# Terence-23/RayTracing-in-a-weekend

Measured on AMD Instinct MI355X. Metric: Msamples/s (rays x bounces) at 1920x1080x500spp, higher is better.
Workload: dtype f32

## Files before the change

bindings/rust/src/lib.rs:

```rust
use std::os::raw::c_void;

#[repr(C)] #[derive(Clone, Copy, Default)]
pub struct RtwCamera { pub origin: [f32; 3], pub u: [f32; 3], pub v: [f32; 3], pub pixel00: [f32; 3],
    pub delta_u: [f32; 3], pub delta_v: [f32; 3], pub lens_radius: f32, pub time0: f32, pub shutter: f32 }

#[repr(C)] #[derive(Clone, Copy, Default)]
pub struct RtwSphere { pub center: [f32; 3], pub radius: f32, pub velocity: [f32; 3], pub col_mod: [f32; 3],
    pub tex_color: [f32; 3], pub metallicness: f32, pub opacity: f32, pub ir: f32, pub emitted: [f32; 3], pub tex: i32 }

#[repr(C)] #[derive(Clone, Copy, Default)]
pub struct RtwTexture { pub row: u32, pub col: u32, pub texel_offset: u32, pub emit_tex: u32 }

#[repr(C)] #[derive(Clone, Copy, Default)]
pub struct RtwQuad { pub origin: [f32; 3], pub u: [f32; 3], pub v: [f32; 3], pub velocity: [f32; 3], pub tex_color: [f32; 3],
    pub metallicness: f32, pub opacity: f32, pub ir: f32, pub emitted: [f32; 3], pub tex: i32 }

#[repr(C)] #[derive(Clone, Copy, Default)]
pub struct RtwTriangle { pub origin: [f32; 3], pub u: [f32; 3], pub v: [f32; 3], pub normal: [f32; 3], pub d: f32, pub w: [f32; 3],
    pub tex_color: [f32; 3], pub metallicness: f32, pub opacity: f32, pub ir: f32, pub emitted: [f32; 3], pub tex: i32 }

#[repr(C)] #[derive(Clone, Copy, Default)]
pub struct RtwMeshInstance { pub position: [f32; 3], pub quat: [f32; 4] }
pub const RTW_MAX_MESH_INSTANCES: u32 = 65536;
pub type MeshHits = (Vec<f32>, Vec<i32>, Vec<i32>, Vec<[f32; 3]>);
// ... 31 lines not shown
    pub total_ms: f32, pub taps: u64 }
#[repr(C)] #[derive(Clone, Copy, Default)]
pub struct RtwGuidedFilter { pub base: RtwBilateral, pub sigma_depth: f32, pub sigma_normal: f32, pub same_object: u32 }
#[repr(u32)] #[derive(Clone, Copy)]
pub enum ProximityKind { Square = 0, Edges = 1 }
#[derive(Clone, Copy)]
pub struct Proximity { pub size: u32, pub kind: ProximityKind }
impl Proximity { pub fn new(size: u32, kind: ProximityKind) -> Self { Self { size, kind } } }

#[repr(C)] pub struct RtwCtx { _private: [u8; 0] }
#[repr(C)] pub struct RtwMgpu { _private: [u8; 0] }

#[repr(u32)] #[derive(Clone, Copy)]
pub enum Integrator { Gradient = 0, BgColor = 1, Normal = 2, Flag = 3, Rust2 = 4, LightCast = 5, LightBiased = 6 }
#[repr(C)] #[derive(Clone, Copy)]
pub struct RtwLight { pub kind: u32, pub index: u32 }
pub const RTW_MAX_LIGHTS: usize = 16;
pub const RTW_FLAG_MIXED_MATERIAL: u32 = 32;
#[repr(u32)] #[derive(Clone, Copy)]
pub enum Sampler { Row = 0, Stratified = 1, Centres = 2, NoRand = 3 }

pub const RTW_OPT_MESH_LIST_MAX: u32 = 12;
pub const RTW_OPT_MESH_CLIMB: u32 = 13;
#[repr(C)]
#[derive(Clone, Copy, Debug, Default)]
pub struct RtwTriNode { pub lo: [f32; 3], pub skip: u32, pub hi: [f32; 3], pub leaf: u32 }

#[repr(C)]
#[derive(Clone, Copy, Debug, Default)]
pub struct RtwSweepRecord { pub a: u32, pub b: u32, pub got: u32, pub reserved: u32 }
#[repr(C)]
#[derive(Clone, Copy, Debug, Default)]
pub struct RtwSweepResult {
    pub tested: u64, pub wrong: u64, pub n_records: u32, pub reserved: u32, pub records: [RtwSweepRecord; 16], pub kernel_ms: f32, pub reserved2: u32,
}
pub const RTW_MATH_SQRT_PLAIN: (u32, u32, u32) = (0, 1, 1);
pub const RTW_MATH_SQRT_IEEE: (u32, u32, u32) = (1, 1, 1);
pub const RTW_MATH_DIV: (u32, u32, u32) = (2, 2, 1);
pub const RTW_MATH_UNIT: (u32, u32, u32) = (3, 3, 3);
pub const RTW_MATH_UNIT_BALL: (u32, u32, u32) = (4, 4, 3);
pub const RTW_MATH_SPHERE_ROOT: (u32, u32, u32) = (5, 4, 1);
pub const RTW_MATH_ATAN2: (u32, u32, u32) = (6, 2, 1);
pub const RTW_MATH_ACOS: (u32, u32, u32) = (7, 1, 1);
pub const RTW_MATH_SPHERE_UV: (u32, u32, u32) = (8, 3, 2);
pub const RTW_MATH_LN: (u32, u32, u32) = (9, 1, 1);
pub const RTW_MATH_POW: (u32, u32, u32) = (10, 2, 1);
// ... 392 lines not shown
```

include/rtw.h:

```cpp
#ifndef RTW_H
#define RTW_H

#include <stdint.h>
#include <stddef.h>

#ifdef __cplusplus
extern "C" {
#endif

#define RTW_ABI_VERSION 4

#define RTW_OK              0
#define RTW_E_INVALID      -1
#define RTW_E_NO_DEVICE    -2
#define RTW_E_HIP          -3
#define RTW_E_NOMEM        -4
#define RTW_E_UNSUPPORTED  -5
#define RTW_E_NO_SCENE     -6
#define RTW_E_INTERNAL     -7
#define RTW_E_RUNTIME_CONFLICT -8

enum {
    RTW_INTEGRATOR_GRADIENT = 0,
    RTW_INTEGRATOR_BG_COLOR = 1,
// ... 147 lines not shown
int  rtw_ctx_set_stream(rtw_ctx *ctx, void *hip_stream);
int  rtw_ctx_set_scene(rtw_ctx *ctx, const RtwScene *scene, float t_begin, float t_end);
int  rtw_ctx_render(rtw_ctx *ctx, const RtwCamera *cam, const RtwParams *params,
                    float *out_rgb, RtwStats *stats);
int  rtw_ctx_render_multi(rtw_ctx *ctx, const RtwCamera *cam, const RtwParams *params, float fps,
                          uint32_t start_frame, uint32_t n_frames, float *out_rgb, RtwStats *stats);
int  rtw_render(const RtwCamera *cam, const RtwScene *scene, const RtwParams *params,
                float *out_rgb, RtwStats *stats);

enum {
    RTW_OPT_CHUNK_LEN        = 1,
    RTW_OPT_SAMPLE_BANK_GB   = 2,
    RTW_OPT_LDS_GEOM         = 3,
    RTW_OPT_BLOCKS_PER_CU    = 4,
    RTW_OPT_LIST_WALK_MAX    = 5,
    RTW_OPT_TILE_ORDER       = 6,
    RTW_OPT_GRAB_BLOCKS      = 7,
    RTW_OPT_TAIL_UNITS       = 9,
    RTW_OPT_SUB_QUEUES       = 8,
    RTW_OPT_GUIDED_LAYOUT    = 10,
    RTW_OPT_NODE_FORMAT      = 11,
    RTW_OPT_MESH_LIST_MAX    = 12,
    RTW_OPT_MESH_CLIMB       = 13,
};
int  rtw_ctx_set_option(rtw_ctx *ctx, uint32_t key, double value);
int  rtw_ctx_last_render_build(rtw_ctx *ctx, char *buf, size_t n);
int  rtw_ctx_last_node_format(rtw_ctx *ctx);
typedef struct RtwRenderFacts {
    uint32_t integrator, sampler, depth, flags, has_textures;
    uint32_t n_quads, n_instances, noise, n_triangles, rotations, placements;
} RtwRenderFacts;
typedef struct RtwTreeFacts { uint32_t n_nodes, depth, n_spheres, has_f16, has_planes; } RtwTreeFacts;
typedef struct RtwRenderChoice {
    char build[32];
    uint32_t node_format, block, lds_stack_off, lds_geom_off, lds_tri_off, lds_bytes;
} RtwRenderChoice;
int  rtw_render_choice(const RtwRenderFacts *request, const RtwTreeFacts *tree, int32_t opt_lds_geom, uint32_t opt_node_format,
                       uint32_t moving, uint32_t accel, RtwRenderChoice *out);

typedef struct rtw_mgpu rtw_mgpu;
int  rtw_mgpu_create(const int *devices, uint32_t n_devices, rtw_mgpu **out);
void rtw_mgpu_destroy(rtw_mgpu *m);
int  rtw_mgpu_set_scene(rtw_mgpu *m, const RtwScene *scene, float t_begin, float t_end);
int  rtw_mgpu_set_option(rtw_mgpu *m, uint32_t key, double value);
int  rtw_mgpu_render(rtw_mgpu *m, const RtwCamera *cam, const RtwParams *params, float *out_rgb,
                     RtwStats *per_device, RtwStats *total);
int  rtw_render_multi_gpu(const int *devices, uint32_t n_devices, const RtwCamera *cam, const RtwScene *scene,
                          const RtwParams *params, float *out_rgb, RtwStats *per_device);

typedef struct RtwPerlin {
    float   ranvec[256][3];
    uint8_t perm_x[256], perm_y[256], perm_z[256];
} RtwPerlin;
typedef struct RtwTextureNoise {
    int32_t perlin;
    float   scale;
} RtwTextureNoise;
int rtw_perlin_new(uint64_t seed, RtwPerlin *out);
int rtw_perlin_eval(const RtwPerlin *t, const float *points, uint32_t n, uint32_t turb_depth, float *out);
int rtw_ctx_perlin_eval(rtw_ctx *ctx, const RtwPerlin *t, const float *points, uint32_t n, uint32_t turb_depth, float *out);
int rtw_ctx_set_texture_noise(rtw_ctx *ctx, const RtwPerlin *tables, uint32_t n_tables,
// ... 231 lines not shown
```

raytracing-in-a-weekend_amd/__init__.py:

```python
from __future__ import annotations

import ctypes as C
import os
from typing import Optional, Sequence

import numpy as np

_HERE = os.path.dirname(os.path.abspath(__file__))
LIB_PATH = os.environ.get("RTW_HIP_LIB", os.path.join(_HERE, "librtw_hip.so"))

RTW_OK = 0
INTEGRATOR_GRADIENT, INTEGRATOR_BG_COLOR, INTEGRATOR_NORMAL, INTEGRATOR_FLAG, INTEGRATOR_RUST2 = 0, 1, 2, 3, 4
INTEGRATOR_LIGHT_CAST, INTEGRATOR_LIGHT_BIASED = 5, 6
LIGHT_SPHERE, LIGHT_QUAD = 0, 1
MAX_LIGHTS = 16
MAX_MESH_INSTANCES = 65536
SAMPLER_ROW, SAMPLER_STRATIFIED, SAMPLER_CENTRES, SAMPLER_NO_RAND = 0, 1, 2, 3
ACCEL_BRUTE, ACCEL_BVH = 0, 1
FLAG_RECURSIVE_ORDER, FLAG_CPP_DIELECTRIC, FLAG_GLOBAL_NODES, FLAG_CPP_DIFFUSE, FLAG_CHUNK_SUMS = 1, 2, 4, 8, 16
FLAG_CPP = FLAG_CPP_DIELECTRIC | FLAG_CPP_DIFFUSE
FLAG_MIXED_MATERIAL = 32
OPT_CHUNK_LEN, OPT_SAMPLE_BANK_GB, OPT_LDS_GEOM, OPT_BLOCKS_PER_CU, OPT_LIST_WALK_MAX, OPT_TILE_ORDER, OPT_GRAB_BLOCKS, OPT_SUB_QUEUES = 1, 2, 3, 4, 5, 6, 7, 8
OPT_TAIL_UNITS = 9
OPT_NODE_FORMAT = 11
NODE_FORMAT_NONE, NODE_FORMAT_F16, NODE_FORMAT_F32 = 0, 1, 2
OPT_MESH_CLIMB = 13
OPT_MESH_LIST_MAX = 12
MESH_LIST_MAX_DEFAULT = 16
OPT_GUIDED_LAYOUT = 10
SCENE_C1, SCENE_C2, SCENE_C4, SCENE_C5, SCENE_METAL_TEST, SCENE_QUAD_TEST, SCENE_PRESENTATION, SCENE_FIRST_FRAME = 1, 2, 4, 5, 6, 7, 8, 9
MEDIUM_SURFACE, MEDIUM_CONST_DENSITY = 0, 1
PROXIMITY_SQUARE, PROXIMITY_EDGES = 0, 1
PIXELS_U8, PIXELS_F32_RUST2 = 0, 1
BILATERAL_MAX_SIZE = 64
STREAM_LEGACY = 1

METALLIC_M = (1.0, 0.0, 1.0)
SCATTER_M = (0.0, 0.0, 1.0)
FUZZY3_M = (0.7, 0.0, 1.0)
GLASS_M = (1.0, 1.0, 1.5)
GLASSR_M = (1.0, 1.0, float(np.float32(1.0) / np.float32(1.5)))
EMPTY_M = SCATTER_M


class RtwError(RuntimeError):
    def __init__(self, status: int, what: str):
        super().__init__(f"{what}: status {status} ({_strerror(status)})")
        self.status = status


class RtwCamera(C.Structure):
# ... 81 lines not shown
class RtwGuidedFilter(C.Structure):
    _fields_ = [("base", RtwBilateral), ("sigma_depth", C.c_float), ("sigma_normal", C.c_float), ("same_object", C.c_uint32)]


class RtwFilterStats(C.Structure):
    _fields_ = [("avg_gradient", C.c_float), ("spatial", C.c_float), ("gradient_ms", C.c_float), ("table_ms", C.c_float),
                ("filter_ms", C.c_float), ("total_ms", C.c_float), ("taps", C.c_uint64)]

    def as_dict(self):
        return {k: getattr(self, k) for k, _ in self._fields_}


class RtwRenderFacts(C.Structure):
    _fields_ = [(k, C.c_uint32) for k in ("integrator", "sampler", "depth", "flags", "has_textures", "n_quads", "n_instances", "noise",
                                          "n_triangles", "rotations", "placements")]


class RtwTreeFacts(C.Structure):
    _fields_ = [(k, C.c_uint32) for k in ("n_nodes", "depth", "n_spheres", "has_f16", "has_planes")]


class RtwRenderChoice(C.Structure):
    _fields_ = [("build", C.c_char * 32)] + [(k, C.c_uint32) for k in ("node_format", "block", "lds_stack_off", "lds_geom_off", "lds_tri_off", "lds_bytes")]


(MATH_SQRT_PLAIN, MATH_SQRT_IEEE, MATH_DIV, MATH_UNIT, MATH_UNIT_BALL, MATH_SPHERE_ROOT, MATH_ATAN2, MATH_ACOS, MATH_SPHERE_UV, MATH_LN, MATH_POW,
 MATH_SINCOS, MATH_EXP) = range(13)
MATH_COLS = {MATH_SQRT_PLAIN: (1, 1), MATH_SQRT_IEEE: (1, 1), MATH_DIV: (2, 1), MATH_UNIT: (3, 3), MATH_UNIT_BALL: (4, 3), MATH_SPHERE_ROOT: (4, 1),
             MATH_ATAN2: (2, 1), MATH_ACOS: (1, 1), MATH_SPHERE_UV: (3, 2), MATH_LN: (1, 1), MATH_POW: (2, 1), MATH_SINCOS: (1, 2), MATH_EXP: (1, 1)}
SWEEP_SQRT, SWEEP_DIV_RANDOM, SWEEP_DIV_MIDPOINT = 0, 1, 2
SWEEP_RECORDS = 16


class RtwSweepRecord(C.Structure):
    _fields_ = [("a", C.c_uint32), ("b", C.c_uint32), ("got", C.c_uint32), ("reserved", C.c_uint32)]


class RtwSweepResult(C.Structure):
    _fields_ = [("tested", C.c_uint64), ("wrong", C.c_uint64), ("n_records", C.c_uint32), ("reserved", C.c_uint32),
                ("records", RtwSweepRecord * SWEEP_RECORDS), ("kernel_ms", C.c_float), ("reserved2", C.c_uint32)]

    def failures(self):
        return [(f"{r.a:#010x}", f"{r.b:#010x}", f"{r.got:#010x}") for r in self.records[:self.n_records]]


_lib = None
# ... 8 lines not shown
                          f"(hipcc --offload-arch=gfx950); there is no CPU fallback")
    L = C.CDLL(LIB_PATH)
    fp = C.POINTER(C.c_float)
    L.rtw_abi_version.restype = C.c_int
    L.rtw_device_count.restype = C.c_int
    L.rtw_strerror.restype = C.c_char_p
    L.rtw_strerror.argtypes = [C.c_int]
    L.rtw_last_hip_error.restype = C.c_int
    L.rtw_ctx_create.argtypes = [C.c_int, C.POINTER(C.c_void_p)]
    L.rtw_ctx_destroy.argtypes = [C.c_void_p]
    L.rtw_ctx_destroy.restype = None
    L.rtw_ctx_set_stream.argtypes = [C.c_void_p, C.c_void_p]
    L.rtw_ctx_set_scene.argtypes = [C.c_void_p, C.POINTER(RtwScene), C.c_float, C.c_float]
    L.rtw_ctx_render.argtypes = [C.c_void_p, C.POINTER(RtwCamera), C.POINTER(RtwParams), C.c_void_p, C.POINTER(RtwStats)]
    L.rtw_ctx_render_multi.argtypes = [C.c_void_p, C.POINTER(RtwCamera), C.POINTER(RtwParams), C.c_float, C.c_uint32, C.c_uint32,
                                       C.c_void_p, C.POINTER(RtwStats)]
    L.rtw_render.argtypes = [C.POINTER(RtwCamera), C.POINTER(RtwScene), C.POINTER(RtwParams), C.c_void_p, C.POINTER(RtwStats)]
    L.rtw_ctx_set_option.argtypes = [C.c_void_p, C.c_uint32, C.c_double]
    L.rtw_ctx_last_render_build.argtypes = [C.c_void_p, C.c_char_p, C.c_size_t]
    L.rtw_ctx_last_node_format.argtypes = [C.c_void_p]
    if hasattr(L, "rtw_render_choice"):
        L.rtw_render_choice.argtypes = [C.POINTER(RtwRenderFacts), C.POINTER(RtwTreeFacts), C.c_int32, C.c_uint32, C.c_uint32, C.c_uint32,
                                        C.POINTER(RtwRenderChoice)]
    L.rtw_mgpu_create.argtypes = [C.POINTER(C.c_int), C.c_uint32, C.POINTER(C.c_void_p)]
    L.rtw_mgpu_destroy.argtypes = [C.c_void_p]
    L.rtw_mgpu_destroy.restype = None
    L.rtw_mgpu_set_scene.argtypes = [C.c_void_p, C.POINTER(RtwScene), C.c_float, C.c_float]
    L.rtw_mgpu_set_option.argtypes = [C.c_void_p, C.c_uint32, C.c_double]
    L.rtw_mgpu_render.argtypes = [C.c_void_p, C.POINTER(RtwCamera), C.POINTER(RtwParams), C.c_void_p, C.POINTER(RtwStats), C.POINTER(RtwStats)]
    L.rtw_render_multi_gpu.argtypes = [C.POINTER(C.c_int), C.c_uint32, C.POINTER(RtwCamera), C.POINTER(RtwScene), C.POINTER(RtwParams),
                                       C.c_void_p, C.POINTER(RtwStats)]
    L.rtw_viewport_new.argtypes = [C.c_uint32, C.c_float, fp, fp, fp, fp, fp, C.POINTER(RtwCamera), C.POINTER(C.c_uint32)]
    L.rtw_viewport_new_from_res.argtypes = [C.c_uint32, C.c_uint32, fp, fp, fp, fp, fp, C.POINTER(RtwCamera), C.POINTER(C.c_uint32)]
    L.rtw_sphere_new.argtypes = [fp, C.c_float, fp, fp, fp, C.POINTER(RtwSphere)]
    L.rtw_sphere_new_with_texture.argtypes = [fp, C.c_float, fp, fp, fp, C.c_int32, C.POINTER(RtwSphere)]
    L.rtw_vec3_rotated.restype = None
    L.rtw_vec3_rotated.argtypes = [fp, fp, fp]
    L.rtw_tile_order.argtypes = [C.c_uint32, C.c_uint32, C.c_uint32, C.POINTER(RtwCamera), C.POINTER(RtwScene), C.POINTER(C.c_uint32), C.c_uint32]
    L.rtw_part_rows.restype = C.c_uint32
    L.rtw_part_rows.argtypes = [C.c_uint32] * 4
    L.rtw_quantize_u8.restype = None
    L.rtw_quantize_u8.argtypes = [fp, C.c_size_t, C.POINTER(C.c_uint8)]
    L.rtw_camera2_new.argtypes = [C.c_float, fp, fp, fp, C.c_float, C.c_float, C.POINTER(RtwCamera)]
    L.rtw_quantize_u8_rust2.restype = None
    L.rtw_quantize_u8_rust2.argtypes = [fp, C.c_size_t, C.POINTER(C.c_uint8)]
    L.rtw_scene_to_json.restype = C.c_size_t
# ... 230 lines not shown


def light_term(integrator: int, pdf, e, t, direction, weight, S, count):
    s = _f3(S)
    c = C.c_float(float(count))
    rc = lib().rtw_light_term(int(integrator), float(pdf), _f3(e), float(t), _f3(direction), float(weight), s, C.byref(c))
    if rc < 0:
        _check(rc, "rtw_light_term")
    return bool(rc), np.array(list(s), np.float32), np.float32(c.value)


def mixed(exp: float):
    return (0.0, -1.0, float(exp))


def render_choice(request: RtwRenderFacts, tree: RtwTreeFacts, lds_geom: int = -1, node_format: int = 0, moving: bool = False,
                  accel: int = ACCEL_BVH) -> dict:
    out = RtwRenderChoice()
    _check(lib().rtw_render_choice(C.byref(request), C.byref(tree), int(lds_geom), int(node_format), 1 if moving else 0, int(accel), C.byref(out)),
           "rtw_render_choice")
    return {"build": out.build.decode(), **{k: int(getattr(out, k)) for k, _ in RtwRenderChoice._fields_[1:]}}


def mixed_validate(scene: "Scene", params: "RtwParams", n_triangles: int = 0, texture_noise: bool = False) -> int:
    return int(lib().rtw_mixed_validate(C.byref(scene.pod), C.byref(params), int(n_triangles), 1 if texture_noise else 0))


def mixed_dir(exp, xi_phi, xi_cos, n) -> np.ndarray:
    out = (C.c_float * 3)()
    _check(lib().rtw_mixed_dir(float(exp), float(xi_phi), float(xi_cos), _f3(n), out), "rtw_mixed_dir")
    return np.array(list(out), np.float32)


def mixed_pdf(exp, p, n, dir_in, ray_o, ray_d) -> np.float32:
    out = C.c_float()
    _check(lib().rtw_mixed_pdf(float(exp), _f3(p), _f3(n), _f3(dir_in), _f3(ray_o), _f3(ray_d), C.byref(out)), "rtw_mixed_pdf")
    return np.float32(out.value)


def _quat_array(quats):
    if quats is None or len(quats) == 0:
        return None, 0, None
    arr = np.ascontiguousarray(quats, np.float32)
    assert arr.ndim == 2 and arr.shape[1] == 4, "quaternions are [n][4] = w, x, y, z"
    return arr.ctypes.data_as(C.POINTER(C.c_float)), len(arr), arr

# ... 1070 lines not shown
```

raytracing-in-a-weekend_amd/csrc/rtw_host.cpp:

```cpp
#include "rtw_host.h"

#include <algorithm>
#include <cfloat>
#include <cmath>
#include <cstring>
#include <limits>

static_assert(sizeof(RtwCamera) == 84 && sizeof(RtwSphere) == 80 && sizeof(RtwTexture) == 16 && sizeof(RtwQuad) == 88, "POD layout");
static_assert(sizeof(RtwInstance) == 48 && sizeof(RtwScene) == 96 && sizeof(RtwParams) == 72 && sizeof(RtwStats) == 160, "POD layout");

namespace rtw {

uint32_t sampler_count(uint32_t sampler, uint32_t samples, uint32_t *s_root) {
    uint32_t root = 0, n = samples;
    if (sampler == RTW_SAMPLER_STRATIFIED) { root = (uint32_t)std::ceil(std::sqrt((float)samples)); n = root * root; }
    else if (sampler == RTW_SAMPLER_CENTRES) { root = (uint32_t)std::floor(std::sqrt((float)samples)); n = root * root; }
    else if (sampler == RTW_SAMPLER_NO_RAND) n = 1;
    if (s_root) *s_root = root;
    return n;
}

namespace {

struct V { float x, y, z; };
// ... 706 lines not shown
                            bool triangles) {
    LdsLayout L{ 0, 0u, RTW_BLOCK, 0u, 0u, 0u, 0u };
    if (bvh) {
        const bool ldsn = t.has_f16 && !global_nodes;
        const uint32_t levels = std::max(t.depth + 3u, 4u), geom_bytes = t.n_spheres * 16u;
        if (ldsn) L.stack_off = lds_align16(t.n_nodes * 32u);
        const uint32_t end = L.stack_off + lds_stack_bytes(levels, RTW_BLOCK, ldsn ? 2u : 4u);
        bool geom_lds = end + geom_bytes <= RTW_CU_LDS_BYTES / RTW_LDS_SHARE_GEOM;
        if (opt_lds_geom >= 0) geom_lds = opt_lds_geom != 0 && t.n_spheres <= RTW_LDS_GEOM_MAX;
        geom_lds = geom_lds && ldsn && !geom && opt_node_format != 2u;
        L.nodes = ldsn ? 1 : 0; L.node_format = ldsn ? 1u : 0u; L.bytes = end;
        if (ldsn && large && !geom_lds) {
            const uint32_t planes = t.n_nodes * RTW_NODE32_DWORDS * 4u, need = planes + lds_stack_bytes(levels, RTW_BLOCK_LARGE, 2u);
            if (t.has_planes && (opt_node_format == 2u ? need <= RTW_CU_LDS_BYTES : (opt_node_format == 0u && 2u * need <= RTW_CU_LDS_BYTES))) {
                L.node_format = 2u; L.block = RTW_BLOCK_LARGE; L.stack_off = planes; L.bytes = need;
            } else geom_lds = true;
        }
        if (geom_lds) { L.nodes = 2; L.geom_off = end; L.bytes = end + geom_bytes; }
    }
    if (triangles) { L.tri_off = lds_align16(L.bytes); L.bytes = L.tri_off + 16u; }
    return L;
}

void build_bvh(const RtwSphere *spheres, uint32_t n, float t_begin, float t_end, BvhBuild &out, const BvhBuildOptions &opt) {
    out.nodes.clear(); out.nodes16.clear(); out.big.clear();
    out.root = std::numeric_limits<int32_t>::min();
    out.centre[0] = out.centre[1] = out.centre[2] = 0.0f;
    out.centre_radius = 0.0f; out.r_min = 0.0f; out.r_max = 0.0f; out.abs_max = 0.0f; out.depth = 0; out.depth_cap = RTW_BVH_STACK;
    if (n == 0) return;

    std::vector<float> radii(n);
    for (uint32_t i = 0; i < n; i++) radii[i] = std::fabs(spheres[i].radius);
    std::vector<float> sorted = radii;
    std::nth_element(sorted.begin(), sorted.begin() + n / 2, sorted.end());
    const float r_med = sorted[n / 2];
    std::vector<uint32_t> order(n);
    for (uint32_t i = 0; i < n; i++) order[i] = i;
    std::stable_sort(order.begin(), order.end(), [&](uint32_t a, uint32_t b) { return radii[a] > radii[b]; });
    std::vector<char> is_big(n, 0);
    if (n > 2) {
        for (uint32_t k = 0; k < n && out.big.size() < RTW_MAX_BIG; k++) {
            uint32_t i = order[k];
            if (!(radii[i] >= 16.0f * r_med) && std::isfinite(radii[i])) break;
            is_big[i] = 1; out.big.push_back(i);
        }
    }
// ... 375 lines not shown
```

raytracing-in-a-weekend_amd/csrc/rtw_host.h:

```cpp
#pragma once
#include <cstdint>
#include <string>
#include <vector>
#include "rtw.h"

namespace rtw {

static inline float host_mul(float a, float b) { return a * b; }
static inline float host_div(float a, float b) { return a / b; }

uint32_t sampler_count(uint32_t sampler, uint32_t samples, uint32_t *s_root);

struct BvhNode {
    float lo0[3], hi0[3];
    float lo1[3], hi1[3];
    int32_t c0, c1;
    uint32_t pad[2];
};
static_assert(sizeof(BvhNode) == 64, "BvhNode must be 64 bytes");

struct BvhNode16 {
    uint16_t plane[2][3][2];
    int16_t c0, c1;
    uint32_t pad;
// ... 38 lines not shown
uint32_t bvh_depth_cap(uint32_t n_leaves, uint32_t n_spheres, bool lds_candidate);

void build_bvh(const RtwSphere *spheres, uint32_t n, float t_begin, float t_end, BvhBuild &out, const BvhBuildOptions &opt = BvhBuildOptions());

void pack_nodes32(const std::vector<BvhNode16> &nodes16, std::vector<uint32_t> &out);

#ifndef RTW_BLOCK
#define RTW_BLOCK 256
#endif
#define RTW_BLOCK_LARGE 768
#define RTW_CU_LDS_BYTES (160u * 1024u)
#define RTW_LDS_SHARE_TREE 7u
#define RTW_LDS_SHARE_GEOM 6u
static inline uint32_t lds_align16(uint32_t bytes) { return (bytes + 15u) & ~15u; }
static inline uint32_t lds_stack_bytes(uint32_t levels, uint32_t block, uint32_t entry_bytes) { return lds_align16(levels * block * entry_bytes); }

struct RenderNeed { int spec; bool geom; };
RenderNeed render_need(const RtwRenderFacts &f);

struct LdsLayout { int nodes; uint32_t node_format, block, stack_off, geom_off, tri_off, bytes; };
LdsLayout render_lds_layout(const RtwTreeFacts &t, int opt_lds_geom, uint32_t opt_node_format, bool bvh, bool global_nodes, bool geom, bool large,
                            bool triangles);

struct HostHit { int32_t sphere; float t; uint32_t node_visits, leaf_tests; };
HostHit bvh_closest_host(const BvhBuild &bb, const RtwSphere *spheres, uint32_t n, const float o[3], const float d[3], float time,
                         float mint, float maxt, bool use_tree, std::string *ops = nullptr);


struct SceneCull {
    float big[16][4];
    uint32_t n_big = 0;
    uint32_t has_tree = 0;
    float lo[3] = { 0, 0, 0 }, hi[3] = { 0, 0, 0 };
    uint32_t n_other = 0;
};
void scene_cull_from_bvh(const BvhBuild &bb, const RtwSphere *spheres, SceneCull &out);
struct TileOrderKey {
    uint32_t mode, tiles_x, tiles_y, k_base, row_block, part_index, part_count, scene_serial, tail_tiles;
    RtwCamera cam;
};
void build_tile_order(uint32_t mode, uint32_t tiles_x, uint32_t tiles_y, uint32_t k_base, uint32_t row_block, uint32_t part_index,
                      uint32_t part_count, const RtwCamera &cam, const SceneCull &cull, uint32_t tail_tiles, std::vector<uint32_t> &order);

}
```

raytracing-in-a-weekend_amd/csrc/rtw_shim.hip:

```cpp
#include "rtw_kernels.h"
#include "rtw_mesh.h"
#include "rtw_refit.h"
#include "rtw_host.h"
#include "rtw_filter.h"
#include "rtw_devmem.h"
#include "rtw_exp.h"
#include "rtw_probe.h"

#include <link.h>

#include <chrono>
#include <cmath>
#include <cstdio>
#include <cstdlib>
#include <cstring>
#include <limits>
#include <map>
#include <new>
#include <utility>
#include <vector>

using namespace rtw;

static thread_local int g_last_hip = 0;
// ... 19 lines not shown
struct QuatMem { DevMem rows; };
struct MeshMem {
    DevMem rows, top;
    DevMem order, first, poses, counts;
};
#define MOVE_POSE_BYTES (7 * sizeof(float))
struct ScratchMem {
    DevMem queue, stats;
    PinnedMem h_stats;
    PinnedMem h_refit;
    DevMem qstats; PinnedMem h_qstats;
    DevMem out;
    PinnedMem h_out;
    DevMem order;
    DevMem samples;
};

struct rtw_ctx {
    int device = 0;
    int n_cu = 0;
    hipStream_t own_stream = nullptr, stream = nullptr;
    hipEvent_t ev0 = nullptr, ev1 = nullptr;
    hipEvent_t ev_mark = nullptr;
    bool has_scene = false;
    bool has_textures = false;
    bool bvh_ok = true;
    double scene_span = 0.0;
    float t_begin = 0.0f, t_end = 0.0f;
    DevScene sc{};
    float bg[3] = { 0, 0, 0 };
    DevGeom geom{};
    DevBvh bvh{};
    const uint32_t *nodes32 = nullptr;
    SceneMem scene_mem;
    uint32_t n_textures = 0;
    std::vector<uint8_t> tex_used;
    bool noise_active = false;
    DevNoise noise{};
    NoiseMem noise_mem;
    FilterScratch *filter = nullptr;
    DevTris tris{};
    bool tri_tree = false;
    TriNode tri_root{};
    TriMem tri_mem;
    bool tri_root_stale = false;
    std::vector<uint32_t> refit_first;
// ... 10 lines not shown
    uint32_t n_mesh_top = 0;
    bool mesh_top_ok = false;
    uint32_t n_top_nodes = 0;
    std::vector<uint32_t> move_first;
    bool tri_textured = false;
    MeshMem mesh_mem;
    bool has_mixed = false, mixed_bad = false;
    ScratchMem scr;
    TileOrderKey order_key{};
    SceneCull cull{};
    uint32_t scene_serial = 0;
    uint32_t opt_chunk_len = 0;
    uint64_t opt_bank_bytes = 48ull << 30;
    int opt_lds_geom = -1;
    uint32_t opt_blocks_per_cu = 0;
    uint32_t opt_list_walk_max = RTW_LIST_WALK_MAX_DEFAULT;
    uint32_t opt_mesh_list_max = RTW_MESH_LIST_MAX_DEFAULT;
    uint32_t opt_mesh_climb = 0;
    uint32_t opt_tile_order = 0;
    uint32_t opt_sub_queues = 0;
    double opt_tail_units = 0.0;
    uint32_t opt_guided_layout = 0;
    uint32_t opt_node_format = 0;
    uint32_t opt_grab_blocks = 2;

    RenderBuild last_build{};
    bool has_last_build = false;
    uint32_t last_node_format = 0;
    std::map<const void *, uint32_t> lds_allowed;
    std::map<std::pair<const void *, uint32_t>, uint32_t> occupancy;
    bool attr_on_device = false; int attr_device = -1;
    struct Pending {
        bool active = false;
        bool marked = false;
        uint32_t n_rows = 0;
        std::chrono::steady_clock::time_point t0;
        float enqueue_ms = 0.0f;
        float *dst = nullptr; bool scatter = false, direct = false, staged = false;
        uint32_t width = 0, height = 0, row_block = 1, part_index = 0, part_count = 1;
        size_t out_bytes = 0;
    } pend;
};

struct OutSpec {
    float *base;
    bool scatter;
// ... 82 lines not shown
    case RTW_E_INTERNAL: return "a render kernel gave up (internal error): the image is incomplete";
    case RTW_E_RUNTIME_CONFLICT: return "two copies of the HIP runtime (libamdhip64) are loaded in this process -- typically PyTorch imported AFTER the first rtw_* call: "
                                        "import torch before using this library (the runtimes then share one copy), or link both against the same runtime";
    default: return "unknown status";
    }
}

int rtw_ctx_create(int device, rtw_ctx **out) {
    if (!out) return RTW_E_INVALID;
    *out = nullptr;
    if (rtw_hip_runtime_count() > 1) return RTW_E_RUNTIME_CONFLICT;
    int n = rtw_device_count();
    if (n <= 0 || device < 0 || device >= n) return RTW_E_NO_DEVICE;
    rtw_ctx *c = new (std::nothrow) rtw_ctx();
    if (!c) return RTW_E_NOMEM;
    c->device = device;
    hipError_t e = hipSetDevice(device);
    hipDeviceProp_t prop;
    if (e == hipSuccess) e = hipGetDeviceProperties(&prop, device);
    if (e == hipSuccess) { c->n_cu = prop.multiProcessorCount; e = hipStreamCreateWithFlags(&c->own_stream, hipStreamNonBlocking); }
    if (e == hipSuccess) e = hipEventCreate(&c->ev0);
    if (e == hipSuccess) e = hipEventCreate(&c->ev1);
    if (e == hipSuccess) e = hipEventCreate(&c->ev_mark);
    if (e == hipSuccess) e = c->scr.queue.reserve(RTW_QUEUE_BYTES);
    if (e == hipSuccess) e = c->scr.stats.reserve(RTW_N_STATS * sizeof(unsigned long long));
    if (e == hipSuccess) e = c->scr.h_stats.reserve(RTW_N_STATS * sizeof(unsigned long long));
    if (e == hipSuccess) e = c->scr.qstats.reserve(RTW_QUERY_SLOTS * RTW_QUERY_STRIDE * sizeof(unsigned long long));
    if (e == hipSuccess) e = c->scr.h_qstats.reserve(RTW_QUERY_SLOTS * RTW_QUERY_STRIDE * sizeof(unsigned long long));
    if (e != hipSuccess) { g_last_hip = (int)e; rtw_ctx_destroy(c); return RTW_E_HIP; }
    c->stream = c->own_stream;
    *out = c;
    return RTW_OK;
}

static void free_noise(rtw_ctx *c) {
    c->noise_mem = NoiseMem{};
    c->noise = DevNoise{};
    c->noise_active = false;
}

static void free_mesh(rtw_ctx *c) {
    c->mesh_mem = MeshMem{};
    c->mesh_rows = nullptr;
    c->n_mesh = 0;
    c->mesh_top = nullptr;
    c->n_mesh_top = 0;
    c->mesh_top_ok = false;
// ... 19 lines not shown
static void free_scene(rtw_ctx *c) {
    c->scene_mem = SceneMem{};
    free_noise(c);
    free_tris(c);
    free_quats(c);
    c->h_instances.clear();
    c->lights = DevLights{};
    c->h_spheres.clear(); c->h_quads.clear(); c->has_medium = false;
    c->has_mixed = c->mixed_bad = false;
    c->n_textures = 0;
    c->tex_used.clear();
    c->has_scene = false;
}

void rtw_ctx_destroy(rtw_ctx *c) {
    if (!c) return;
    (void)hipSetDevice(c->device);
    free_scene(c);
    c->scr = ScratchMem{};
    filter_scratch_free(c->filter);
    if (c->ev_mark) (void)hipEventDestroy(c->ev_mark);
    if (c->ev0) (void)hipEventDestroy(c->ev0);
    if (c->ev1) (void)hipEventDestroy(c->ev1);
    if (c->own_stream) (void)hipStreamDestroy(c->own_stream);
    delete c;
}

int rtw_ctx_set_stream(rtw_ctx *c, void *hip_stream) {
    if (!c) return RTW_E_INVALID;
    c->stream = hip_stream ? (hipStream_t)hip_stream : c->own_stream;
    return RTW_OK;
}

static void scene_mixed(const RtwScene *s, bool &has_mixed, bool &mixed_bad) {
    has_mixed = mixed_bad = false;
    auto see = [&](float opacity, float ir) {
        if (!(opacity < 0.0f)) return;
        has_mixed = true;
        if (!(ir >= 0.0f && ir <= 3.402823466e38f)) mixed_bad = true;
    };
    for (uint32_t i = 0; i < s->n_spheres; i++) see(s->spheres[i].opacity, s->spheres[i].ir);
    for (uint32_t i = 0; i < s->n_quads; i++) see(s->quads[i].opacity, s->quads[i].ir);
    for (uint32_t i = 0; i < s->n_inst_spheres; i++) see(s->inst_spheres[i].opacity, s->inst_spheres[i].ir);
    for (uint32_t i = 0; i < s->n_inst_quads; i++) see(s->inst_quads[i].opacity, s->inst_quads[i].ir);
}
static int mixed_check(uint32_t flags, uint32_t integrator, bool has_mixed, bool mixed_bad, bool noise, bool tris, bool medium) {
// ... 1021 lines not shown
    }
    uint32_t per_cu = c->opt_blocks_per_cu;
    if (per_cu == 0) {
        const auto key = std::make_pair((const void *)fn, a.lds_bytes);
        auto it = c->occupancy.find(key);
        if (it == c->occupancy.end()) {
            int n = 0;
            if (hipOccupancyMaxActiveBlocksPerMultiprocessor(&n, (const void *)fn, (int)block, a.lds_bytes) != hipSuccess || n < 1) n = 1;
            it = c->occupancy.emplace(key, (uint32_t)(n > 8 ? 8 : n)).first;
        }
        per_cu = it->second;
    }

    if (!(phases & PH_LAUNCH)) return RTW_OK;

    if (!c->pend.marked) HIP_TRY(hipEventRecord(c->ev_mark, c->stream));
    HIP_TRY(hipMemsetAsync(a.stats, 0, RTW_N_STATS * sizeof(unsigned long long), c->stream));
#ifdef RTW_ENDTIMES
    HIP_TRY(hipMemsetAsync(a.stats + 24, 0xFF, sizeof(unsigned long long), c->stream));
    HIP_TRY(hipMemsetAsync(a.stats + 26, 0xFF, sizeof(unsigned long long), c->stream));
    HIP_TRY(hipMemsetAsync(a.stats + 28, 0xFF, sizeof(unsigned long long), c->stream));
#endif
    HIP_TRY(hipEventRecord(c->ev0, c->stream));
    for (uint32_t tr0 = 0; tr0 < tile_rows || tr0 == 0; tr0 += (uint32_t)band_tile_rows) {
        const uint32_t tr1 = tr0 + (uint32_t)band_tile_rows < tile_rows ? tr0 + (uint32_t)band_tile_rows : tile_rows;
        a.k_base = tr0 * 8; a.k_end = tr1 * 8 < n_rows ? tr1 * 8 : n_rows;
        a.n_tiles = a.tiles_x * (tr1 - tr0);
        a.total_work = a.n_tiles * a.n_chunks * 64u;
        a.reg_q1 = a.reg_q2 = a.n_tiles;
        for (int r = 0; r < 3; r++) { a.reg_len[r] = a.chunk_len; a.reg_nc[r] = a.n_chunks; }
        a.tile_order = nullptr;
        if (c->opt_tile_order && a.n_tiles > 2u && !((c->opt_tile_order == 2u || c->opt_tile_order == 5u) && c->cull.n_other)) {
            const uint32_t tiles_y = a.n_tiles / a.tiles_x;
            TileOrderKey key;
            std::memset(&key, 0, sizeof key);
            key.mode = c->opt_tile_order; key.tiles_x = a.tiles_x; key.tiles_y = tiles_y; key.k_base = a.k_base;
            key.row_block = a.row_block; key.part_index = a.part_index; key.part_count = a.part_count; key.cam = *cam; key.scene_serial = c->scene_serial;
            key.cam.time0 = key.cam.shutter = key.cam.lens_radius = 0.0f;
            const uint64_t per_tile = 64ull * a.n_chunks;
            key.tail_tiles = (uint32_t)std::min<uint64_t>(a.n_tiles, ((uint64_t)c->n_cu * per_cu * block * 4ull + per_tile - 1) / per_tile);
            if (!c->scr.order.ptr || std::memcmp(&key, &c->order_key, sizeof key) != 0) {
                std::vector<uint32_t> order;
                build_tile_order(c->opt_tile_order, a.tiles_x, tiles_y, a.k_base, a.row_block, a.part_index, a.part_count, *cam, c->cull, key.tail_tiles, order);
                HIP_TRY(c->scr.order.reserve(order.size() * sizeof(uint32_t)));
                HIP_TRY(hipMemcpyAsync(c->scr.order.ptr, order.data(), order.size() * sizeof(uint32_t), hipMemcpyHostToDevice, c->stream));
                HIP_TRY(hipStreamSynchronize(c->stream));
                c->order_key = key;
            }
// ... 11 lines not shown
            const uint32_t need = (a.total_work + block - 1) / block;
            if (grid > need) grid = need ? need : 1;
        }
        if (!sums && c->opt_tail_units > 0.0 && a.chunk_len > 1u && a.n_tiles > 1u) {
            const double waves = (double)grid * (block / 64u);
            const uint32_t L1 = a.chunk_len, L2 = L1 >= 12u ? 4u : (L1 >= 6u ? 2u : 1u), L3 = 1u;
            uint64_t t3 = (uint64_t)std::ceil(c->opt_tail_units * waves * L3 / (double)a.n_samples);
            uint64_t t2 = L2 > L3 ? (uint64_t)std::ceil(c->opt_tail_units * waves * L2 / (double)a.n_samples) : 0;
            if (t3 > a.n_tiles / 4u) t3 = a.n_tiles / 4u;
            if (t2 > a.n_tiles / 4u) t2 = a.n_tiles / 4u;
            a.reg_q2 = a.n_tiles - (uint32_t)t3; a.reg_q1 = a.reg_q2 - (uint32_t)t2;
            a.reg_len[1] = L2; a.reg_len[2] = L3;
            for (int r = 1; r < 3; r++) a.reg_nc[r] = (a.n_samples + a.reg_len[r] - 1u) / a.reg_len[r];
            a.total_work = (a.reg_q1 * a.reg_nc[0] + (a.reg_q2 - a.reg_q1) * a.reg_nc[1] + (a.n_tiles - a.reg_q2) * a.reg_nc[2]) * 64u;
        }
        {
            a.sub_shift = (c->opt_sub_queues != 1u && a.n_tiles >= 64u && grid >= 64u) ? RTW_SUB_SHIFT : 0u;
            const uint32_t waves4 = (grid * (block / 64u) * 4u) >> a.sub_shift;
            a.grab_shift = 0; while (a.grab_shift < 31u && (1u << a.grab_shift) < waves4) a.grab_shift++;
            uint32_t blocks = c->opt_grab_blocks ? c->opt_grab_blocks : a.n_chunks;
            if (blocks > a.n_chunks) blocks = a.n_chunks;
            a.grab_max = (blocks ? blocks : 1u) * 64u;
        }
        HIP_TRY(hipMemsetAsync(a.queue, 0, RTW_QUEUE_BYTES, c->stream));
        if (a.n_tiles) { launch_render(fn, block, a, grid, c->stream); c->last_build = build; c->has_last_build = true; c->last_node_format = lds.node_format; }
        HIP_TRY(hipGetLastError());
        if (tile_rows == 0) break;
    }
    HIP_TRY(hipEventRecord(c->ev1, c->stream));
    HIP_TRY(hipMemcpyAsync(c->scr.h_stats.ptr, a.stats, RTW_N_STATS * sizeof(unsigned long long), hipMemcpyDeviceToHost, c->stream));
    c->pend.active = true; c->pend.n_rows = n_rows;
    c->pend.dst = out.base; c->pend.scatter = out.scatter; c->pend.direct = direct; c->pend.staged = staged;
    c->pend.width = p->width; c->pend.height = p->height; c->pend.row_block = a.row_block; c->pend.part_index = p->part_index; c->pend.part_count = p->part_count;
    c->pend.out_bytes = out_bytes;
    c->pend.enqueue_ms = std::chrono::duration<float, std::milli>(std::chrono::steady_clock::now() - c->pend.t0).count();
    if (phases & PH_COPY) return render_copy(c);
    return RTW_OK;
}

static int render_copy(rtw_ctx *c) {
    if (!c || !c->pend.active) return RTW_E_INVALID;
    const rtw_ctx::Pending &q = c->pend;
    if (q.direct) return RTW_OK;
    HIP_TRY(hipSetDevice(c->device));
    if (q.staged) {
        HIP_TRY(hipMemcpyAsync(c->scr.h_out.ptr, c->scr.out.ptr, q.out_bytes, hipMemcpyDeviceToHost, c->stream));
    } else if (q.scatter) {
        const int rc = scatter_rows(c, c->scr.out.as<float>(), q.dst, q.width, q.height, q.row_block, q.part_index, q.part_count);
        if (rc != RTW_OK) return rc;
    } else HIP_TRY(hipMemcpyAsync(q.dst, c->scr.out.ptr, q.out_bytes, hipMemcpyDefault, c->stream));
// ... 78 lines not shown
    return len > 0 && (size_t)len < n ? RTW_OK : RTW_E_INVALID;
}

int rtw_ctx_last_render_build(rtw_ctx *c, char *buf, size_t n) {
    if (!c || !buf || n == 0 || !c->has_last_build) return RTW_E_INVALID;
    return print_build(c->last_build, buf, n);
}

int rtw_render_choice(const RtwRenderFacts *f, const RtwTreeFacts *t, int32_t opt_lds_geom, uint32_t opt_node_format, uint32_t moving, uint32_t accel,
                      RtwRenderChoice *out) {
    if (!f || !t || !out || accel > RTW_ACCEL_BVH || opt_lds_geom < -1 || opt_lds_geom > 1 || opt_node_format > 2u) return RTW_E_INVALID;
    const RenderChoice choice = render_choice(*f, *t, opt_lds_geom, opt_node_format, moving != 0u, accel == RTW_ACCEL_BVH);
    if (!choice.fn) return RTW_E_UNSUPPORTED;
    const LdsLayout &lds = choice.lds;
    *out = RtwRenderChoice{ {}, lds.node_format, lds.block, lds.stack_off, lds.geom_off, lds.tri_off, lds.bytes };
    return print_build(choice.build, out->build, sizeof out->build);
}

int rtw_ctx_last_node_format(rtw_ctx *c) {
    if (!c || !c->has_last_build) return RTW_E_INVALID;
    return (int)c->last_node_format;
}

uint32_t rtw_mesh_list_max_default(void) { return RTW_MESH_LIST_MAX_DEFAULT; }

int rtw_ctx_set_option(rtw_ctx *c, uint32_t key, double v) {
    if (!c || !(v == v)) return RTW_E_INVALID;
    switch (key) {
    case RTW_OPT_CHUNK_LEN:      if (!(v >= 0.0 && v <= 255.0)) return RTW_E_INVALID; c->opt_chunk_len = (uint32_t)v; return RTW_OK;
    case RTW_OPT_SAMPLE_BANK_GB: if (!(v > 0.0 && v <= 1048576.0)) return RTW_E_INVALID; c->opt_bank_bytes = (uint64_t)(v * (double)(1ull << 30)); return RTW_OK;
    case RTW_OPT_LDS_GEOM:       if (!(v >= -1.0 && v <= 1.0)) return RTW_E_INVALID; c->opt_lds_geom = (int)v; return RTW_OK;
    case RTW_OPT_BLOCKS_PER_CU:  if (!(v >= 0.0 && v <= 8.0)) return RTW_E_INVALID; c->opt_blocks_per_cu = (uint32_t)v; return RTW_OK;
    case RTW_OPT_LIST_WALK_MAX:  if (!(v >= 0.0 && v <= 4294967295.0)) return RTW_E_INVALID; c->opt_list_walk_max = (uint32_t)v; return RTW_OK;
    case RTW_OPT_TILE_ORDER:     if (!(v >= 0.0 && v <= 5.0 && v == (double)(uint32_t)v)) return RTW_E_INVALID; c->opt_tile_order = (uint32_t)v; return RTW_OK;
    case RTW_OPT_SUB_QUEUES:     if (!(v == 0.0 || v == 1.0)) return RTW_E_INVALID; c->opt_sub_queues = (uint32_t)v; return RTW_OK;
    case RTW_OPT_TAIL_UNITS:     if (!(v >= 0.0 && v <= 1024.0)) return RTW_E_INVALID; c->opt_tail_units = v; return RTW_OK;
    case RTW_OPT_GUIDED_LAYOUT:  if (!(v >= 0.0 && v <= 4.0 && v == (double)(uint32_t)v)) return RTW_E_INVALID; c->opt_guided_layout = (uint32_t)v; return RTW_OK;
    case RTW_OPT_GRAB_BLOCKS:    if (!(v >= 0.0 && v <= 65536.0 && v == (double)(uint32_t)v)) return RTW_E_INVALID; c->opt_grab_blocks = (uint32_t)v; return RTW_OK;
    case RTW_OPT_MESH_LIST_MAX:  if (!(v >= 0.0 && v <= 4294967295.0 && v == (double)(uint32_t)v)) return RTW_E_INVALID; c->opt_mesh_list_max = (uint32_t)v; return RTW_OK;
    case RTW_OPT_MESH_CLIMB:     if (!(v == 0.0 || v == 1.0 || v == 2.0)) return RTW_E_INVALID; c->opt_mesh_climb = (uint32_t)v; return RTW_OK;
    case RTW_OPT_NODE_FORMAT:    if (!(v == 0.0 || v == 1.0 || v == 2.0)) return RTW_E_INVALID; c->opt_node_format = (uint32_t)v; return RTW_OK;
    default: return RTW_E_INVALID;
    }
}

int rtw_ctx_render(rtw_ctx *c, const RtwCamera *cam, const RtwParams *p, float *out_rgb, RtwStats *stats) {
    int rc = render_enqueue(c, cam, p, OutSpec{ out_rgb, false });
    if (rc != RTW_OK) return rc;
    return render_wait(c, stats);
}

int rtw_mgpu_create(const int *devices, uint32_t n, rtw_mgpu **out) {
    if (!out) return RTW_E_INVALID;
    *out = nullptr;
    if (!devices || n == 0 || n > 64) return RTW_E_INVALID;
    if (rtw_device_count() <= 0) return RTW_E_NO_DEVICE;
    rtw_mgpu *m = new (std::nothrow) rtw_mgpu();
    if (!m) return RTW_E_NOMEM;
    for (uint32_t k = 0; k < n; k++) {
        rtw_ctx *c = nullptr;
        int rc = rtw_ctx_create(devices[k], &c);
        if (rc != RTW_OK) { rtw_mgpu_destroy(m); return rc; }
        m->ctx.push_back(c);
    }
// ... 152 lines not shown
```

Before: 40720.

## Split last tile rows onto a low-priority side stream to fill the tail

Result: no change. 40970, median of 6 (+0.6%).

```diff
diff --git a/bindings/rust/src/lib.rs b/bindings/rust/src/lib.rs
--- a/bindings/rust/src/lib.rs
+++ b/bindings/rust/src/lib.rs
@@ -77,6 +77,7 @@
 
 pub const RTW_OPT_MESH_LIST_MAX: u32 = 12;
 pub const RTW_OPT_MESH_CLIMB: u32 = 13;
+pub const RTW_OPT_TAIL_ROWS: u32 = 14;
 #[repr(C)]
 #[derive(Clone, Copy, Debug, Default)]
 pub struct RtwTriNode { pub lo: [f32; 3], pub skip: u32, pub hi: [f32; 3], pub leaf: u32 }
diff --git a/include/rtw.h b/include/rtw.h
--- a/include/rtw.h
+++ b/include/rtw.h
@@ -193,6 +193,7 @@
     RTW_OPT_NODE_FORMAT      = 11,
     RTW_OPT_MESH_LIST_MAX    = 12,
     RTW_OPT_MESH_CLIMB       = 13,
+    RTW_OPT_TAIL_ROWS        = 14,
 };
 int  rtw_ctx_set_option(rtw_ctx *ctx, uint32_t key, double value);
 int  rtw_ctx_last_render_build(rtw_ctx *ctx, char *buf, size_t n);
@@ -208,6 +209,13 @@
 } RtwRenderChoice;
 int  rtw_render_choice(const RtwRenderFacts *request, const RtwTreeFacts *tree, int32_t opt_lds_geom, uint32_t opt_node_format,
                        uint32_t moving, uint32_t accel, RtwRenderChoice *out);
+typedef struct RtwTailSplitFacts {
+    uint32_t tile_rows, n_cu, wg_per_cu, block;
+    uint64_t total_work;
+    uint32_t bands, chunk_sums, tile_order, multi_gpu;
+    int32_t  opt_tail_rows;
+} RtwTailSplitFacts;
+uint32_t rtw_render_tail_split(const RtwTailSplitFacts *facts);
 
 typedef struct rtw_mgpu rtw_mgpu;
 int  rtw_mgpu_create(const int *devices, uint32_t n_devices, rtw_mgpu **out);
diff --git a/raytracing-in-a-weekend_amd/__init__.py b/raytracing-in-a-weekend_amd/__init__.py
--- a/raytracing-in-a-weekend_amd/__init__.py
+++ b/raytracing-in-a-weekend_amd/__init__.py
@@ -27,6 +27,7 @@
 OPT_MESH_CLIMB = 13
 OPT_MESH_LIST_MAX = 12
 MESH_LIST_MAX_DEFAULT = 16
+OPT_TAIL_ROWS = 14
 OPT_GUIDED_LAYOUT = 10
 SCENE_C1, SCENE_C2, SCENE_C4, SCENE_C5, SCENE_METAL_TEST, SCENE_QUAD_TEST, SCENE_PRESENTATION, SCENE_FIRST_FRAME = 1, 2, 4, 5, 6, 7, 8, 9
 MEDIUM_SURFACE, MEDIUM_CONST_DENSITY = 0, 1
@@ -154,6 +155,11 @@
 
 class RtwRenderChoice(C.Structure):
     _fields_ = [("build", C.c_char * 32)] + [(k, C.c_uint32) for k in ("node_format", "block", "lds_stack_off", "lds_geom_off", "lds_tri_off", "lds_bytes")]
+
+
+class RtwTailSplitFacts(C.Structure):
+    _fields_ = ([(k, C.c_uint32) for k in ("tile_rows", "n_cu", "wg_per_cu", "block")] + [("total_work", C.c_uint64)]
+                + [(k, C.c_uint32) for k in ("bands", "chunk_sums", "tile_order", "multi_gpu")] + [("opt_tail_rows", C.c_int32)])
 
 
 (MATH_SQRT_PLAIN, MATH_SQRT_IEEE, MATH_DIV, MATH_UNIT, MATH_UNIT_BALL, MATH_SPHERE_ROOT, MATH_ATAN2, MATH_ACOS, MATH_SPHERE_UV, MATH_LN, MATH_POW,
@@ -208,6 +214,9 @@
     if hasattr(L, "rtw_render_choice"):
         L.rtw_render_choice.argtypes = [C.POINTER(RtwRenderFacts), C.POINTER(RtwTreeFacts), C.c_int32, C.c_uint32, C.c_uint32, C.c_uint32,
                                         C.POINTER(RtwRenderChoice)]
+    if hasattr(L, "rtw_render_tail_split"):
+        L.rtw_render_tail_split.argtypes = [C.POINTER(RtwTailSplitFacts)]
+        L.rtw_render_tail_split.restype = C.c_uint32
     L.rtw_mgpu_create.argtypes = [C.POINTER(C.c_int), C.c_uint32, C.POINTER(C.c_void_p)]
     L.rtw_mgpu_destroy.argtypes = [C.c_void_p]
     L.rtw_mgpu_destroy.restype = None
@@ -484,6 +493,13 @@
     return {"build": out.build.decode(), **{k: int(getattr(out, k)) for k, _ in RtwRenderChoice._fields_[1:]}}
 
 
+def render_tail_split(tile_rows: int, total_work: int, tail_rows: int = -1, n_cu: int = 256, wg_per_cu: int = 2, block: int = 768, bands: int = 1,
+                      chunk_sums: bool = False, tile_order: bool = False, multi_gpu: bool = False) -> int:
+    f = RtwTailSplitFacts(int(tile_rows), int(n_cu), int(wg_per_cu), int(block), int(total_work), int(bands), 1 if chunk_sums else 0,
+                          1 if tile_order else 0, 1 if multi_gpu else 0, int(tail_rows))
+    return int(lib().rtw_render_tail_split(C.byref(f)))
+
+
 def mixed_validate(scene: "Scene", params: "RtwParams", n_triangles: int = 0, texture_noise: bool = False) -> int:
     return int(lib().rtw_mixed_validate(C.byref(scene.pod), C.byref(params), int(n_triangles), 1 if texture_noise else 0))
 
diff --git a/raytracing-in-a-weekend_amd/csrc/rtw_host.cpp b/raytracing-in-a-weekend_amd/csrc/rtw_host.cpp
--- a/raytracing-in-a-weekend_amd/csrc/rtw_host.cpp
+++ b/raytracing-in-a-weekend_amd/csrc/rtw_host.cpp
@@ -752,6 +752,19 @@
     return L;
 }
 
+uint32_t render_tail_split(const RtwTailSplitFacts &f) {
+    if (f.opt_tail_rows == 0 || f.tile_rows < 2u || f.bands != 1u || f.chunk_sums || f.tile_order || f.multi_gpu) return 0u;
+    uint64_t k = (uint64_t)f.opt_tail_rows;
+    if (f.opt_tail_rows < 0) {
+        if (f.n_cu == 0u || f.wg_per_cu == 0u || f.block == 0u) return 0u;
+        if (f.total_work / f.n_cu / f.wg_per_cu / f.block < RTW_TAIL_MIN_ITEMS_PER_LANE) return 0u;
+        if (f.tile_rows < 16u * RTW_TAIL_ROWS_AUTO) return 0u;
+        k = RTW_TAIL_ROWS_AUTO;
+    }
+    if (k > f.tile_rows - 1u) k = f.tile_rows - 1u;
+    return f.tile_rows - (uint32_t)k;
+}
+
 void build_bvh(const RtwSphere *spheres, uint32_t n, float t_begin, float t_end, BvhBuild &out, const BvhBuildOptions &opt) {
     out.nodes.clear(); out.nodes16.clear(); out.big.clear();
     out.root = std::numeric_limits<int32_t>::min();
diff --git a/raytracing-in-a-weekend_amd/csrc/rtw_host.h b/raytracing-in-a-weekend_amd/csrc/rtw_host.h
--- a/raytracing-in-a-weekend_amd/csrc/rtw_host.h
+++ b/raytracing-in-a-weekend_amd/csrc/rtw_host.h
@@ -84,6 +84,10 @@
 LdsLayout render_lds_layout(const RtwTreeFacts &t, int opt_lds_geom, uint32_t opt_node_format, bool bvh, bool global_nodes, bool geom, bool large,
                             bool triangles);
 
+#define RTW_TAIL_ROWS_AUTO 5u
+#define RTW_TAIL_MIN_ITEMS_PER_LANE 150u
+uint32_t render_tail_split(const RtwTailSplitFacts &f);
+
 struct HostHit { int32_t sphere; float t; uint32_t node_visits, leaf_tests; };
 HostHit bvh_closest_host(const BvhBuild &bb, const RtwSphere *spheres, uint32_t n, const float o[3], const float d[3], float time,
                          float mint, float maxt, bool use_tree, std::string *ops = nullptr);
diff --git a/raytracing-in-a-weekend_amd/csrc/rtw_shim.hip b/raytracing-in-a-weekend_amd/csrc/rtw_shim.hip
--- a/raytracing-in-a-weekend_amd/csrc/rtw_shim.hip
+++ b/raytracing-in-a-weekend_amd/csrc/rtw_shim.hip
@@ -65,6 +65,8 @@
     hipStream_t own_stream = nullptr, stream = nullptr;
     hipEvent_t ev0 = nullptr, ev1 = nullptr;
     hipEvent_t ev_mark = nullptr;
+    hipStream_t side_stream = nullptr;
+    hipEvent_t ev_fork = nullptr, ev_join = nullptr;
     bool has_scene = false;
     bool has_textures = false;
     bool bvh_ok = true;
@@ -121,6 +123,7 @@
     double opt_tail_units = 0.0;
     uint32_t opt_guided_layout = 0;
     uint32_t opt_node_format = 0;
+    int32_t opt_tail_rows = -1;
     uint32_t opt_grab_blocks = 2;
 
     RenderBuild last_build{};
@@ -249,7 +252,7 @@
     if (e == hipSuccess) e = hipEventCreate(&c->ev0);
     if (e == hipSuccess) e = hipEventCreate(&c->ev1);
     if (e == hipSuccess) e = hipEventCreate(&c->ev_mark);
-    if (e == hipSuccess) e = c->scr.queue.reserve(RTW_QUEUE_BYTES);
+    if (e == hipSuccess) e = c->scr.queue.reserve(2u * RTW_QUEUE_BYTES);
     if (e == hipSuccess) e = c->scr.stats.reserve(RTW_N_STATS * sizeof(unsigned long long));
     if (e == hipSuccess) e = c->scr.h_stats.reserve(RTW_N_STATS * sizeof(unsigned long long));
     if (e == hipSuccess) e = c->scr.qstats.reserve(RTW_QUERY_SLOTS * RTW_QUERY_STRIDE * sizeof(unsigned long long));
@@ -315,6 +318,9 @@
     if (c->ev_mark) (void)hipEventDestroy(c->ev_mark);
     if (c->ev0) (void)hipEventDestroy(c->ev0);
     if (c->ev1) (void)hipEventDestroy(c->ev1);
+    if (c->ev_fork) (void)hipEventDestroy(c->ev_fork);
+    if (c->ev_join) (void)hipEventDestroy(c->ev_join);
+    if (c->side_stream) (void)hipStreamDestroy(c->side_stream);
     if (c->own_stream) (void)hipStreamDestroy(c->own_stream);
     delete c;
 }
@@ -1382,8 +1388,7 @@
     HIP_TRY(hipMemsetAsync(a.stats + 28, 0xFF, sizeof(unsigned long long), c->stream));
 #endif
     HIP_TRY(hipEventRecord(c->ev0, c->stream));
-    for (uint32_t tr0 = 0; tr0 < tile_rows || tr0 == 0; tr0 += (uint32_t)band_tile_rows) {
-        const uint32_t tr1 = tr0 + (uint32_t)band_tile_rows < tile_rows ? tr0 + (uint32_t)band_tile_rows : tile_rows;
+    auto launch_rows = [&](KArgs a, uint32_t tr0, uint32_t tr1, hipStream_t s, bool zero_queue) -> int {
         a.k_base = tr0 * 8; a.k_end = tr1 * 8 < n_rows ? tr1 * 8 : n_rows;
         a.n_tiles = a.tiles_x * (tr1 - tr0);
         a.total_work = a.n_tiles * a.n_chunks * 64u;
@@ -1441,10 +1446,49 @@
             if (blocks > a.n_chunks) blocks = a.n_chunks;
             a.grab_max = (blocks ? blocks : 1u) * 64u;
         }
-        HIP_TRY(hipMemsetAsync(a.queue, 0, RTW_QUEUE_BYTES, c->stream));
-        if (a.n_tiles) { launch_render(fn, block, a, grid, c->stream); c->last_build = build; c->has_last_build = true; c->last_node_format = lds.node_format; }
+        if (zero_queue) HIP_TRY(hipMemsetAsync(a.queue, 0, RTW_QUEUE_BYTES, s));
+        if (a.n_tiles) { launch_render(fn, block, a, grid, s); c->last_build = build; c->has_last_build = true; c->last_node_format = lds.node_format; }
         HIP_TRY(hipGetLastError());
-        if (tile_rows == 0) break;
+        return RTW_OK;
+    };
+    RtwTailSplitFacts split{};
+    split.tile_rows = tile_rows; split.n_cu = (uint32_t)c->n_cu; split.wg_per_cu = per_cu; split.block = block;
+    split.total_work = (uint64_t)a.tiles_x * tile_rows * a.n_chunks * 64ull;
+    split.bands = band_tile_rows ? (uint32_t)((tile_rows + band_tile_rows - 1) / band_tile_rows) : 1u;
+    split.chunk_sums = sums; split.tile_order = c->opt_tile_order != 0u; split.multi_gpu = out.scatter || phases != PH_ALL;
+    split.opt_tail_rows = c->opt_tail_rows;
+    if (const uint32_t tail_row = render_tail_split(split)) {
+        if (!c->side_stream) {
+            int least = 0, greatest = 0;
+            HIP_TRY(hipDeviceGetStreamPriorityRange(&least, &greatest));
+            HIP_TRY(hipStreamCreateWithPriority(&c->side_stream, hipStreamNonBlocking, least));
+        }
+        if (!c->ev_fork) HIP_TRY(hipEventCreateWithFlags(&c->ev_fork, hipEventDisableTiming));
+        if (!c->ev_join) HIP_TRY(hipEventCreateWithFlags(&c->ev_join, hipEventDisableTiming));
+        HIP_TRY(hipMemsetAsync(a.queue, 0, 2u * RTW_QUEUE_BYTES, c->stream));
+        HIP_TRY(hipEventRecord(c->ev_fork, c->stream));
+        HIP_TRY(hipStreamWaitEvent(c->side_stream, c->ev_fork, 0));
+        int rc = launch_rows(a, 0u, tail_row, c->stream, false);
+        if (rc == RTW_OK) {
+            KArgs t = a;
+            t.samples += (size_t)tail_row * slots_per_tile_row * 3u;
+            t.queue += RTW_QUEUE_BYTES / sizeof(uint32_t);
+            rc = launch_rows(t, tail_row, tile_rows, c->side_stream, false);
+        }
+        const int keep = g_last_hip;
+        hipError_t e = hipEventRecord(c->ev_join, c->side_stream);
+        if (e == hipSuccess) e = hipStreamWaitEvent(c->stream, c->ev_join, 0);
+        if (e != hipSuccess) {
+            if (hipStreamSynchronize(c->side_stream) != hipSuccess) (void)hipGetLastError();
+            if (rc == RTW_OK) { g_last_hip = (int)e; rc = RTW_E_HIP; } else g_last_hip = keep;
+        }
+        if (rc != RTW_OK) return rc;
+    } else {
+        for (uint32_t tr0 = 0; tr0 < tile_rows || tr0 == 0; tr0 += (uint32_t)band_tile_rows) {
+            const uint32_t tr1 = tr0 + (uint32_t)band_tile_rows < tile_rows ? tr0 + (uint32_t)band_tile_rows : tile_rows;
+            if (const int rc = launch_rows(a, tr0, tr1, c->stream, true)) return rc;
+            if (tile_rows == 0) break;
+        }
     }
     HIP_TRY(hipEventRecord(c->ev1, c->stream));
     HIP_TRY(hipMemcpyAsync(c->scr.h_stats.ptr, a.stats, RTW_N_STATS * sizeof(unsigned long long), hipMemcpyDeviceToHost, c->stream));
@@ -1569,6 +1613,8 @@
     return (int)c->last_node_format;
 }
 
+uint32_t rtw_render_tail_split(const RtwTailSplitFacts *f) { return f ? render_tail_split(*f) : 0u; }
+
 uint32_t rtw_mesh_list_max_default(void) { return RTW_MESH_LIST_MAX_DEFAULT; }
 
 int rtw_ctx_set_option(rtw_ctx *c, uint32_t key, double v) {
@@ -1587,6 +1633,7 @@
     case RTW_OPT_MESH_LIST_MAX:  if (!(v >= 0.0 && v <= 4294967295.0 && v == (double)(uint32_t)v)) return RTW_E_INVALID; c->opt_mesh_list_max = (uint32_t)v; return RTW_OK;
     case RTW_OPT_MESH_CLIMB:     if (!(v == 0.0 || v == 1.0 || v == 2.0)) return RTW_E_INVALID; c->opt_mesh_climb = (uint32_t)v; return RTW_OK;
     case RTW_OPT_NODE_FORMAT:    if (!(v == 0.0 || v == 1.0 || v == 2.0)) return RTW_E_INVALID; c->opt_node_format = (uint32_t)v; return RTW_OK;
+    case RTW_OPT_TAIL_ROWS:      if (!(v >= -1.0 && v <= 65535.0 && v == (double)(int32_t)v)) return RTW_E_INVALID; c->opt_tail_rows = (int32_t)v; return RTW_OK;
     default: return RTW_E_INVALID;
     }
 }
```
